# QingYunA/General-Medical-Image-Segmentation-CNN-Framework

Hardware: AMD Instinct MI355X
Metric: train voxels/sec (128^3 patches) 3D U-Net (higher is better)
Workload: dtype f32 (f16x3 split MFMA: every fp32 conv operand = two fp16 parts under a per-tensor power-of-two scale, three fp16 products per fp32 product, fp32 accumulate; graded against fp64 by the same tests as bf16x6 and the exact-fp32 MFMA path); 1 GPU; unet3d_f32_2x128: UNet3D(1,2,32) fwd+BCE+bwd+Adam+Dice, x=[2,1,128,128,128] fp32 per GPU, random-init (kaiming) weights, data-parallel replicas with RCCL gradient all-reduce, conv math f16x3; global_batch=2, parallelism=dp1, conv_math=f16x3, optimizer=torch.optim.Adam(fused=True)

## Files before the change

general-medical-image-segmentation-cnn-framework_amd/csrc/conv_mfma.hip:

```cpp
#include "common.h"
#include "internal.h"
#include "igemm_kernel.h"
#include "pack.h"
#include <stdlib.h>
#include <initializer_list>

namespace seg {

__global__ void pack_wq_kernel(const float* __restrict__ w, float* __restrict__ wq, int K, int Nn, int T, int NT, int mode, int aux, int CK,
                               int TW, TapList taps, const float* __restrict__ oscale) {
    const long long total = (long long)K * Nn * T;
    for (long long idx = (long long)blockIdx.x * blockDim.x + threadIdx.x; idx < total; idx += (long long)gridDim.x * blockDim.x) {
        long long r = idx;
        int s = (int)(r % 4); r /= 4;
        int j = (int)(r % NT); r /= NT;
        int h = (int)(r % 2); r /= 2;
        int kk = (int)(r % (CK / 8)); r /= (CK / 8);
        int tap = (int)(r % T); r /= T;
        int chunk = (int)(r % (K / CK)); r /= (K / CK);
        int nt = (int)r;
        wq[idx] = pack_src(w, mode, nt * NT + j, chunk * CK + kk * 8 + h * 4 + s, tap, K, Nn, T, aux, TW, taps) * (oscale ? oscale[nt * NT + j] : 1.f);
    }
}

__global__ void pack_wq_x3s_kernel(const float* __restrict__ w, bf16* __restrict__ wq, int K, int Nn, int NBW, int mode, const float* __restrict__ oscale) {
    const int NT = 32 * NBW, NU = X3S_NPAIR * NBW, nch = K / 16;
    const long long total = (long long)(Nn / NT) * nch * NU * 1024;
    for (long long idx = (long long)blockIdx.x * blockDim.x + threadIdx.x; idx < total; idx += (long long)gridDim.x * blockDim.x) {
        long long q = idx;
        const int e = (int)(q % 8); q /= 8;
        const int lane = (int)(q % 64); q /= 64;
        const int t2 = (int)(q % 2); q /= 2;
        const int u = (int)(q % NU); q /= NU;
        const int chunk = (int)(q % nch); q /= nch;
        const int nt = (int)q;
        const int s = u / NBW, nh = u % NBW, g = lane >> 4, c = lane & 15;
        const int tap = x3s_pair_tap(s, g >> 1);
        const int co = nt * NT + nh * 32 + t2 * 16 + c;
        const float v = tap < 27 ? pack_src(w, mode, co, chunk * 16 + 8 * (g & 1) + e, tap, K, Nn, 27, 0, 27, TapList{}) * (oscale ? oscale[co] : 1.f) : 0.f;
        bf16 bh, bm, bl;
        split3(v, bh, bm, bl);
        const long long base = (((long long)nt * nch + chunk) * NU + u) * 3072 + t2 * 512 + lane * 8 + e;
        wq[base] = bh; wq[base + 1024] = bm; wq[base + 2048] = bl;
    }
}

__global__ void pack_wq_x3s_f16_kernel(const float* __restrict__ w, _Float16* __restrict__ wq, int K, int Nn, int NBW, int mode, const float* __restrict__ oscale,
                                       const float* __restrict__ amax_w) {
    const int NT = 32 * NBW, NU = X3S_NPAIR * NBW, nch = K / 16;
    const long long total = (long long)(Nn / NT) * nch * NU * 1024;
    const float sc = pow2f(f16x_scale_exp(*amax_w));
    for (long long idx = (long long)blockIdx.x * blockDim.x + threadIdx.x; idx < total; idx += (long long)gridDim.x * blockDim.x) {
        long long q = idx;
        const int e = (int)(q % 8); q /= 8;
        const int lane = (int)(q % 64); q /= 64;
        const int t2 = (int)(q % 2); q /= 2;
        const int u = (int)(q % NU); q /= NU;
        const int chunk = (int)(q % nch); q /= nch;
        const int nt = (int)q;
        const int s = u / NBW, nh = u % NBW, g = lane >> 4, c = lane & 15;
        const int tap = x3s_pair_tap(s, g >> 1);
        const int co = nt * NT + nh * 32 + t2 * 16 + c;
        const float v = tap < 27 ? pack_src(w, mode, co, chunk * 16 + 8 * (g & 1) + e, tap, K, Nn, 27, 0, 27, TapList{}) * (oscale ? oscale[co] : 1.f) * sc : 0.f;
        _Float16 bh, bl;
        split2h(v, bh, bl);
        const long long base = (((long long)nt * nch + chunk) * NU + u) * 2048 + t2 * 512 + lane * 8 + e;
        wq[base] = bh; wq[base + 1024] = bl;
    }
}

__global__ __launch_bounds__(256) void amax_kernel(const float* __restrict__ x, int ld, long long rows, int C, const float* __restrict__ rowscale, unsigned* __restrict__ slot) {
    float m = 0.f;
    if ((C % 4) == 0 && (ld % 4) == 0 && ((uintptr_t)x % 16) == 0) {
        const int cw = C / 4;
        const long long total = rows * cw;
        for (long long idx = (long long)blockIdx.x * 256 + threadIdx.x; idx < total; idx += (long long)gridDim.x * 256) {
            const long long r = idx / cw;
            const f32x4_t v = *reinterpret_cast<const f32x4_t*>(x + r * ld + (idx - r * cw) * 4);
            const float sc = rowscale ? fabsf(rowscale[r]) : 1.f;
            m = fmaxf(m, fmaxf(fmaxf(fabsf(v[0]), fabsf(v[1])), fmaxf(fabsf(v[2]), fabsf(v[3]))) * sc);
        }
    } else {
        const long long total = rows * C;
        for (long long idx = (long long)blockIdx.x * 256 + threadIdx.x; idx < total; idx += (long long)gridDim.x * 256) {
            const long long r = idx / C;
            m = fmaxf(m, fabsf(x[r * ld + (idx - r * C)]) * (rowscale ? fabsf(rowscale[r]) : 1.f));
        }
    }
#pragma unroll
    for (int o = 32; o > 0; o >>= 1) m = fmaxf(m, __shfl_xor(m, o, 64));
    __shared__ float sh[4];
    if ((threadIdx.x & 63) == 0) sh[threadIdx.x >> 6] = m;
    __syncthreads();
    if (threadIdx.x == 0) {
        m = fmaxf(fmaxf(sh[0], sh[1]), fmaxf(sh[2], sh[3]));
        atomicMax(slot, __builtin_bit_cast(unsigned, m));
    }
}
void tensor_amax(const float* x, int ld, long long rows, int C, const float* rowscale, float* slot, hipStream_t st) {
    const long long work = rows * (long long)C / 4;
    const int grid = (int)(work / 1024 < 1 ? 1 : (work / 1024 > 2048 ? 2048 : work / 1024));
    hipLaunchKernelGGL(amax_kernel, dim3(grid), dim3(256), 0, st, x, ld, rows, C, rowscale, reinterpret_cast<unsigned*>(slot));
}

__global__ void pack_wq_b16s_kernel(const float* __restrict__ w, bf16* __restrict__ wq, int K, int Nn, int T, int NT, int mode, const float* __restrict__ oscale) {
    const int nstep = (T + 1) / 2, nch = K / 16, ntt = NT / 16;
    const long long total = (long long)(Nn / NT) * nch * nstep * ntt * 512;
    for (long long idx = (long long)blockIdx.x * blockDim.x + threadIdx.x; idx < total; idx += (long long)gridDim.x * blockDim.x) {
        long long q = idx;
        const int e = (int)(q % 8); q /= 8;
        const int lane = (int)(q % 64); q /= 64;
        const int tt = (int)(q % ntt); q /= ntt;
        const int s = (int)(q % nstep); q /= nstep;
        const int chunk = (int)(q % nch); q /= nch;
        const int nt = (int)q;
        const int g = lane >> 4, c = lane & 15;
        const int tap = 2 * s + (g >> 1);
        const int co = nt * NT + 32 * (tt >> 1) + 8 * (c >> 2) + 4 * (tt & 1) + (c & 3);
        wq[idx] = tap < T ? (bf16)(pack_src(w, mode, co, chunk * 16 + 8 * (g & 1) + e, tap, K, Nn, T, 0, T, TapList{}) * (oscale ? oscale[co] : 1.f)) : (bf16)0.f;
    }
// ... 592 lines not shown
```

general-medical-image-segmentation-cnn-framework_amd/csrc/conv_x3s.hip:

```cpp
#include "common.h"
#include "internal.h"
#include "igemm_kernel.h"
#include <type_traits>

namespace seg {

namespace {

#ifndef X3S_WN2
#define X3S_WN2 1
#endif
#ifndef X3S_WD
#define X3S_WD 3
#endif
#ifndef X3S_XD
#define X3S_XD 2
#endif
#ifndef X3S_HALO_AUX
#define X3S_HALO_AUX 0
#endif
#ifndef X3S_SPLIT_MIX
#define X3S_SPLIT_MIX 0
#endif
#ifndef X3S_BNX_EARLY
#define X3S_BNX_EARLY 1
#endif
constexpr int XBX = 16, XTY = 4, XHX = XBX + 2, XHY = XTY + 2;
constexpr int X3S_PRO_MAX_CIN = 512;

template <int LW, bool F16 = false, int WN = 1>
struct Geo {
    static constexpr int NPL = F16 ? 2 : 3;
    static constexpr int LINES = (4 / WN) * LW, TZ = LINES / XTY, HZ = TZ + 2;
    static constexpr int NVOX = XHX * XHY * HZ;
    static constexpr int PS = (NVOX + 15) / 16 * 16;
    static constexpr int LDS_BYTES = 2 * NPL * PS * 16;
    static constexpr int NPIECE = NVOX * 4;
    static constexpr int NITER = (NPIECE + 255) / 256;
};


__device__ __forceinline__ constexpr int tap_slot(int t) { return ((t / 9) * XHY + (t / 3) % 3) * XHX + t % 3; }
__device__ __forceinline__ constexpr int pair_kind(int s) { return s < 9 ? 0 : (s < 12 ? 1 : (s == 12 ? 2 : 3)); }

__device__ __forceinline__ float row16_sum(float v) {
    v += __builtin_bit_cast(float, __builtin_amdgcn_update_dpp(0, __builtin_bit_cast(int, v), 0xB1, 0xF, 0xF, true));
    v += __builtin_bit_cast(float, __builtin_amdgcn_update_dpp(0, __builtin_bit_cast(int, v), 0x4E, 0xF, 0xF, true));
    v += __builtin_bit_cast(float, __builtin_amdgcn_update_dpp(0, __builtin_bit_cast(int, v), 0x141, 0xF, 0xF, true));
    v += __builtin_bit_cast(float, __builtin_amdgcn_update_dpp(0, __builtin_bit_cast(int, v), 0x140, 0xF, 0xF, true));
    return v;
}

template <int LW, int NBW, int TZ, int WN = 1>
__device__ __forceinline__ void x3_epilogue(const IgemmArgs& a, f32x4 (&acc)[LW][2 * NBW], int scale_exp, int ks, int mtile, int n, int x0, int y0, int z0,
                                            int n0_tile, int line0, int r, int g, int wave, int tid, unsigned char* lds_raw) {
    constexpr int NT = 32 * NBW, NTW = 2 * NBW;
    constexpr int NTT = NT * WN, WM = 4 / WN;
    const int wn = WN == 1 ? 0 : wave % WN;
    const int n0 = n0_tile + wn * NT;
    const int gx = x0 + r;
    constexpr int LH = (8 / NTW) < LW ? (8 / NTW) : LW;
    constexpr int NG = (LW + LH - 1) / LH;
    constexpr bool DB = NG > 1 && NTW <= 2;
    f32x4 bxv[DB ? 2 : 1][LH][NTW];
    const int bnx_lane = min(gx, a.W - 1) * a.ldbnx + n0 + 4 * g;
    auto load_bnx = [&](int j0, int buf) {
#pragma unroll
        for (int j = 0; j < LH; ++j) {
            const int line = line0 + min(j0 + j, LW - 1);
            const int cz = min(z0 + line / XTY, a.D - 1), cy = min(y0 + line % XTY, a.H - 1);
            const float* src = a.bnx + (((long long)n * a.D + cz) * a.H + cy) * a.W * a.ldbnx + bnx_lane;
#pragma unroll
            for (int t = 0; t < NTW; ++t) bxv[buf][j][t] = *reinterpret_cast<const f32x4*>(src + 16 * t);
        }
    };
    if (a.bnpart) { load_bnx(0, 0); if (DB && X3S_BNX_EARLY) load_bnx(LH, 1); }
    if (scale_exp != 0) {
#pragma unroll
        for (int j = 0; j < LW; ++j)
#pragma unroll
            for (int t = 0; t < NTW; ++t)
#pragma unroll
                for (int e = 0; e < 4; ++e) acc[j][t][e] = __builtin_ldexpf(acc[j][t][e], scale_exp);
    }
    float* yslab = reinterpret_cast<float*>(a.y) + (long long)ks * a.split_stride;
    float* const ylane = yslab + ((((long long)n * a.D + z0) * a.H + y0) * a.W + gx) * a.ldy + n0 + 4 * g;
    float ssum[NTW][4];
#pragma unroll
    for (int t = 0; t < NTW; ++t)
#pragma unroll
        for (int e = 0; e < 4; ++e) ssum[t][e] = 0.f;
    float ymax = 0.f;
    f32x4 bv[NTW];
#pragma unroll
    for (int t = 0; t < NTW; ++t) bv[t] = a.bias ? *reinterpret_cast<const f32x4*>(a.bias + n0 + 16 * t + 4 * g) : f32x4{0.f, 0.f, 0.f, 0.f};
    auto store_lines = [&](auto ACTc) {
// ... 95 lines not shown
            for (int e = 0; e < 4; ++e) {
                const int c = 16 * t + 4 * g + e;
                float sm = 0.f;
#pragma unroll
                for (int w = 0; w < WM; ++w) sm += lds[(w * WN + wn) * NT + c];
                tmean[t][e] = sm / cnt;
            }
        __syncthreads();
        float m2[NTW][4];
#pragma unroll
        for (int t = 0; t < NTW; ++t)
#pragma unroll
            for (int e = 0; e < 4; ++e) m2[t][e] = 0.f;
#pragma unroll
        for (int j = 0; j < LW; ++j) {
            const int line = line0 + j;
            const bool inside = (z0 + line / XTY) < a.D && (y0 + line % XTY) < a.H && gx < a.W;
#pragma unroll
            for (int t = 0; t < NTW; ++t)
#pragma unroll
                for (int e = 0; e < 4; ++e) {
                    const float d = acc[j][t][e] + bv[t][e] - tmean[t][e];
                    if (inside) m2[t][e] += d * d;
                }
        }
#pragma unroll
        for (int t = 0; t < NTW; ++t)
#pragma unroll
            for (int e = 0; e < 4; ++e) {
                const float v = row16_sum(m2[t][e]);
                if (r == 0) lds[(4 + wave) * NT + 16 * t + 4 * g + e] = v;
            }
        __syncthreads();
        if (tid < NTT) {
            const int cw = tid / NT, cl = tid % NT;
            float s1 = 0.f, mm = 0.f;
#pragma unroll
            for (int w = 0; w < WM; ++w) { s1 += lds[(w * WN + cw) * NT + cl]; mm += lds[(4 + w * WN + cw) * NT + cl]; }
            float* dst = a.spart + ((long long)mtile * a.Cout + n0_tile + tid) * 3;
            dst[0] = s1; dst[1] = mm; dst[2] = cnt;
        }
    }
}

template <int LW, int NBW, bool F16, int WN = 1, bool PRO = false>
__global__ __launch_bounds__(256, 2) void conv_x3s_kernel(IgemmArgs a) {
    using G = Geo<LW, F16, WN>;
    constexpr int NPL = G::NPL;
    constexpr int NT = 32 * NBW * WN;
    constexpr int NTW = 2 * NBW;
    constexpr int NU = X3S_NPAIR * NBW;
    constexpr int NUP = X3S_NPAIR * NBW * WN;
    constexpr int UNIT = 2 * NPL * 512;
    constexpr int PS = G::PS;
    extern __shared__ __attribute__((aligned(16))) unsigned char lds_raw[];

    const int tid = threadIdx.x, lane = tid & 63, wave = __builtin_amdgcn_readfirstlane(tid >> 6);
    const int r = lane & 15, g = lane >> 4;

    int ks, ntile, mtile, n, x0, y0, z0;
    {
        const int total = (int)gridDim.x, bid = blockIdx.x;
        const int q8 = total >> 3, r8 = total & 7, xcd = bid & 7;
        const int xstart = xcd < r8 ? xcd * (q8 + 1) : r8 * (q8 + 1) + (xcd - r8) * q8, xcnt = q8 + (xcd < r8 ? 1 : 0);
        const int local = bid >> 3;
        if (local >= xcnt) return;
        int t = xstart + local;
        ks = t % a.ksplit; t /= a.ksplit;
        ntile = t % a.nN;
        mtile = t / a.nN;
        int mt = mtile;
        const int per_n = a.ntx * a.nty * a.ntz;
        n = mt / per_n; mt -= n * per_n;
        const int zfull = a.ntz / a.bz;
        const int rowtiles = a.ntx * a.nty * a.bz;
        int zrow = mt / rowtiles, bzz = a.bz;
        if (zrow >= zfull) { zrow = zfull; bzz = a.ntz - zfull * a.bz; }
        mt -= zrow * rowtiles;
        const int blk = a.ntx * a.by * bzz;
        const int b = mt / blk; mt -= b * blk;
        const int txi = mt % a.ntx; mt /= a.ntx;
        const int tyi = b * a.by + mt % a.by;
        const int tzi = zrow * a.bz + mt / a.by;
        x0 = txi * XBX; y0 = tyi * XTY; z0 = tzi * G::TZ;
    }
    const int n0 = ntile * NT;
    const int c0 = ks * a.cps, c1 = c0 + a.cps;
    const float* __restrict__ xin = reinterpret_cast<const float*>(a.x);
    int sx = 0, sw = 0;
    if constexpr (F16) { sx = f16x_scale_exp(*a.amax_x); sw = f16x_scale_exp(*a.amax_w); }
    const float xscale = pow2f(sx);
    float* const ptab = reinterpret_cast<float*>(lds_raw + G::LDS_BYTES);
    const int pcin = a.nchunks * 16;
    if constexpr (PRO) {
        for (int i = tid; i < pcin; i += 256) { ptab[i] = a.pro_al[i] * xscale; ptab[pcin + i] = a.pro_be[i] * xscale; }
    }

    int voff[G::NITER];
    halo_piece_offsets<G::NITER, G::NPIECE, 4, XHX, XHY, G::HZ>(voff, tid, x0 - 1, y0 - 1, z0 - 1, a.D, a.H, a.W, a.ldx * 4);
    const float* xsample = xin + (long long)n * a.D * a.H * a.W * a.ldx;
    const int sample_bytes = a.D * a.H * a.W * a.ldx * 4;
    f32x4 stage[G::NITER];
    auto load_stage = [&](int chunk) {
        const auto rsrc = __builtin_amdgcn_make_buffer_rsrc(const_cast<float*>(xsample + chunk * 16), 0, sample_bytes, 0x00020000);
#pragma unroll
        for (int it = 0; it < G::NITER; ++it)
// ... 29 lines not shown
#endif
    unsigned char* const wdst = lds_raw + (((tid & 3) >> 1) * PS + (tid >> 2)) * 16 + (tid & 1) * 8;
    auto write_stage = [&](int chunk, auto WPRO, auto MASK, auto RELU) {
        f32x4 pal = {0.f, 0.f, 0.f, 0.f}, pbe = pal;
        if constexpr (decltype(WPRO)::value) {
            pal = *reinterpret_cast<const f32x4*>(ptab + chunk * 16 + (tid & 3) * 4);
            pbe = *reinterpret_cast<const f32x4*>(ptab + pcin + chunk * 16 + (tid & 3) * 4);
        }
#pragma unroll
        for (int it = 0; it < G::NITER; ++it) {
            if (it * 256 + tid < G::NPIECE) {
                using u32x2 = __attribute__((ext_vector_type(2))) unsigned;
                unsigned char* dst = wdst + it * 1024;
                if constexpr (F16) {
                    unsigned h0, l0, h1, l1;
                    if constexpr (decltype(WPRO)::value) {
                        f32x4 v;
#pragma unroll
                        for (int e = 0; e < 4; ++e) {
                            const float z = fmaf(stage[it][e], pal[e], pbe[e]);
                            v[e] = decltype(RELU)::value ? fmaxf(z, 0.f) : fmaxf(z, z * a.pro_slope);
                        }
                        if constexpr (decltype(MASK)::value) { if (voff[it] == 0x7FFFFFF0) v = f32x4{0.f, 0.f, 0.f, 0.f}; }
                        split_pair_h(v[0], v[1], h0, l0, 1.f);
                        split_pair_h(v[2], v[3], h1, l1, 1.f);
                    } else if (SEG_DBG(a, 256)) {
                        using u32x4 = __attribute__((ext_vector_type(4))) unsigned;
                        const u32x4 u = __builtin_bit_cast(u32x4, stage[it]);
                        h0 = u[0]; h1 = u[1]; l0 = u[2]; l1 = u[3];
                    } else {
                        split_pair_h(stage[it][0], stage[it][1], h0, l0, xscale);
                        split_pair_h(stage[it][2], stage[it][3], h1, l1, xscale);
                    }
                    const u32x2 qh = {h0, h1}, ql = {l0, l1};
                    *reinterpret_cast<u32x2*>(dst) = qh;
                    *reinterpret_cast<u32x2*>(dst + 2 * PS * 16) = ql;
                } else {
                    unsigned h0, m0, l0, h1, m1, l1;
                    split_pair(stage[it][0], stage[it][1], h0, m0, l0);
                    split_pair(stage[it][2], stage[it][3], h1, m1, l1);
                    const u32x2 qh = {h0, h1}, qm = {m0, m1}, ql = {l0, l1};
                    *reinterpret_cast<u32x2*>(dst) = qh;
                    *reinterpret_cast<u32x2*>(dst + 2 * PS * 16) = qm;
                    *reinterpret_cast<u32x2*>(dst + 4 * PS * 16) = ql;
                }
            }
        }
    };

    const int wm = WN == 1 ? wave : wave / WN, wn = WN == 1 ? 0 : wave % WN;
    const int line0 = wm * LW;
    const int lane_slot = ((line0 / XTY) * XHY + (line0 % XTY)) * XHX + r + (g & 1) * PS;
    const int hi = g >> 1;
    const int xb0 = (lane_slot + hi) * 16, xb1 = (lane_slot + hi * XHX) * 16, xb2 = (lane_slot + hi * XHY * XHX) * 16, xb3 = lane_slot * 16;
    auto xaddr = [&](int s, int j, int pl) {
        const int base = pair_kind(s) == 0 ? xb0 : (pair_kind(s) == 1 ? xb1 : (pair_kind(s) == 2 ? xb2 : xb3));
        return base + (((j >> 2) * XHY + (j & 3)) * XHX + tap_slot(x3s_pair_tap(s, 0)) + 2 * pl * PS) * 16;
    };

    f32x4 acc[LW][NTW];
#pragma unroll
    for (int j = 0; j < LW; ++j)
#pragma unroll
        for (int t = 0; t < NTW; ++t) acc[j][t] = f32x4{0.f, 0.f, 0.f, 0.f};
    const bool interior = x0 >= 1 && y0 >= 1 && z0 >= 1 && x0 + XBX + 1 <= a.W && y0 + XTY + 1 <= a.H && z0 + G::TZ + 1 <= a.D;

    const bf16* wlane = reinterpret_cast<const bf16*>(a.wq) + (long long)ntile * a.nchunks * (NUP * UNIT) + lane * 8;
    if (!SEG_DBG(a, 1024)) load_stage(c0);
    for (int chunk = c0; chunk < (SEG_DBG(a, 512) ? c0 : c1); ++chunk) {
        const bf16* wp = wlane + (long long)chunk * (NUP * UNIT) + wn * (NBW * UNIT);
        constexpr int WD = F16 ? ((PRO && LW == 8 && WN == 1) ? 2 : X3S_WD) : (NBW == 2 && LW == 4 ? 1 : 2);
        constexpr int XD = F16 ? X3S_XD : 1;
        bf16x8_t wf[WD + 1][2][NPL], xf[XD + 1][NPL];
        auto load_w = [&](int u) {
#pragma unroll
            for (int t2 = 0; t2 < 2; ++t2)
#pragma unroll
                for (int pl = 0; pl < NPL; ++pl) wf[u % (WD + 1)][t2][pl] = *reinterpret_cast<const bf16x8_t*>(wp + ((u / NBW) * (NBW * WN) + u % NBW) * UNIT + (pl * 2 + t2) * 512);
        };
#pragma unroll
        for (int u = 0; u < WD; ++u) load_w(u);
        if (!SEG_DBG(a, 1) || chunk == c0) {
        __syncthreads();
        if (!SEG_DBG(a, 4) || chunk == c0) {
            using TT = std::true_type; using FF = std::false_type;
            if constexpr (!PRO) write_stage(chunk, FF{}, FF{}, FF{});
            else if (a.pro_act == MI355SEG_ACT_RELU) { if (interior) write_stage(chunk, TT{}, FF{}, TT{}); else write_stage(chunk, TT{}, TT{}, TT{}); }
            else write_stage(chunk, TT{}, TT{}, FF{});
        }
        __syncthreads();
        }
        const bool more = chunk + 1 < c1;
#pragma unroll
        for (int q0 = 0; q0 < XD; ++q0)
#pragma unroll
            for (int pl = 0; pl < NPL; ++pl) xf[q0][pl] = *reinterpret_cast<const bf16x8_t*>(lds_raw + xaddr((q0 / LW) / NBW, q0 % LW, pl));
        __builtin_amdgcn_sched_barrier(0);
#pragma unroll
        for (int u = 0; u < NU; ++u) {
            const int s = u / NBW, nh = u % NBW;
#pragma unroll
            for (int j = 0; j < LW; ++j) {
                const int q = u * LW + j, cur = q % (XD + 1), nxt = (q + XD) % (XD + 1);
                if (j == 0 && u + WD < NU && !SEG_DBG(a, 2)) load_w(u + WD);
                if (q < G::NITER && more && !SEG_DBG(a, 1) && !SEG_DBG(a, 16)) load_piece(chunk + 1, q);
                if (q + XD < NU * LW && !SEG_DBG(a, 8)) {
                    const int u2 = (q + XD) / LW, j2 = (q + XD) % LW;
#pragma unroll
                    for (int pl = 0; pl < NPL; ++pl) xf[nxt][pl] = *reinterpret_cast<const bf16x8_t*>(lds_raw + xaddr(u2 / NBW, j2, pl));
                }
                if constexpr (F16) {
                    constexpr int PW[3] = {1, 0, 0}, PX[3] = {0, 1, 0};
#pragma unroll
                    for (int pr = 0; pr < 3; ++pr)
#pragma unroll
                        for (int t2 = 0; t2 < 2; ++t2)
                            acc[j][nh * 2 + t2] = __builtin_amdgcn_mfma_f32_16x16x32_f16(__builtin_bit_cast(f16x8_t, wf[u % (WD + 1)][t2][PW[pr]]),
                                                                                      __builtin_bit_cast(f16x8_t, xf[cur][PX[pr]]), acc[j][nh * 2 + t2], 0, 0, 0);
                } else {
                    constexpr int PW[6] = {2, 0, 1, 1, 0, 0}, PX[6] = {0, 2, 1, 0, 1, 0};
#pragma unroll
                    for (int pr = 0; pr < 6; ++pr)
#pragma unroll
                        for (int t2 = 0; t2 < 2; ++t2)
                            acc[j][nh * 2 + t2] = __builtin_amdgcn_mfma_f32_16x16x32_bf16(wf[u % (WD + 1)][t2][PW[pr]], xf[cur][PX[pr]], acc[j][nh * 2 + t2], 0, 0, 0);
                }
#pragma unroll
                for (int k = 0; k < NPL; ++k) {
                    __builtin_amdgcn_sched_group_barrier(0x100, 1, 0);
                    __builtin_amdgcn_sched_group_barrier(0x008, 1, 0);
                }
                if (j == 0 || q < G::NITER) {
#pragma unroll
                    for (int k = 0; k < 2 * NPL + 1; ++k) {
                        __builtin_amdgcn_sched_group_barrier(0x020, 1, 0);
                        __builtin_amdgcn_sched_group_barrier(0x008, 1, 0);
                    }
                }
                __builtin_amdgcn_sched_barrier(0);
            }
        }
        __builtin_amdgcn_sched_barrier(0);
    }

    x3_epilogue<LW, NBW, G::TZ, WN>(a, acc, F16 ? -(sx + sw) : 0, ks, mtile, n, x0, y0, z0, n0, line0, r, g, wave, tid, lds_raw);
}

template <int LW, int NBW, bool F16, int WN = 1>
void launch_x3s(const IgemmArgs& a, int nwg, hipStream_t st) {
    constexpr int LDSB = Geo<LW, F16, WN>::LDS_BYTES;
    static_assert(LDSB >= 8 * 64 * 4, "the statistics epilogue needs 8 x NT floats");
    if constexpr (F16) {
        if (a.pro_al) {
            SEG_SET_LDS((conv_x3s_kernel<LW, NBW, true, WN, true>), LDSB + X3S_PRO_MAX_CIN * 8);
            hipLaunchKernelGGL((conv_x3s_kernel<LW, NBW, true, WN, true>), dim3(nwg), dim3(256), LDSB + a.nchunks * 16 * 8, st, a);
            return;
        }
    }
    SEG_SET_LDS((conv_x3s_kernel<LW, NBW, F16, WN>), LDSB);
    hipLaunchKernelGGL((conv_x3s_kernel<LW, NBW, F16, WN>), dim3(nwg), dim3(256), LDSB, st, a);
}


template <int NBW>
struct GeoW {
    static constexpr int LW = 8, TZ = 8, HZ = TZ + 2;
    static constexpr int NVOX = XHX * XHY * HZ;
    static constexpr int PS = (NVOX + 15) / 16 * 16;
    static constexpr int BUF = 4 * PS * 16;
    static constexpr int LDS_BYTES = 2 * BUF;
    static constexpr int NPIECE = NVOX * 4;
    static constexpr int NITER = (NPIECE + 255) / 256;
    static constexpr int NCH = NBW == 2 ? 1 : 2;
    static constexpr int WR = NBW == 2 ? 2 : 4, WL = NBW == 2 ? 1 : 2;
    static constexpr int RING = 8;
    static_assert((NCH * X3S_NPAIR) % WR == 0 && WL < WR, "the weight ring's phase must be static");
};

// ... 30 lines not shown
        const int txi = mt % a.ntx; mt /= a.ntx;
        const int tyi = b * a.by + mt % a.by;
        const int tzi = zrow * a.bz + mt / a.by;
        x0 = txi * XBX; y0 = tyi * XTY; z0 = tzi * G::TZ;
    }
    const int n0 = ntile * NT;
    const int c1 = a.cps;
    const float* __restrict__ xin = reinterpret_cast<const float*>(a.x);
    const int sx = f16x_scale_exp(*a.amax_x), sw = f16x_scale_exp(*a.amax_w);
    const float xscale = pow2f(sx);

    int voff[NITER];
#pragma unroll
    for (int it = 0; it < NITER; ++it) {
        const int p = it * 256 + tid;
        const int vox = p >> 2, part = p & 3;
        const int hz = vox / (XHY * XHX), rem = vox % (XHY * XHX);
        const int hy = rem / XHX, hx = rem % XHX;
        const int gz = z0 - 1 + hz, gy = y0 - 1 + hy, gx = x0 - 1 + hx;
        const bool ok = (p < G::NPIECE) && (unsigned)gz < (unsigned)a.D && (unsigned)gy < (unsigned)a.H && (unsigned)gx < (unsigned)a.W;
        voff[it] = ok ? (((gz * a.H + gy) * a.W + gx) * a.ldx + part * 4) * 4 : 0x7FFFFFF0;
    }
    const float* xsample = xin + (long long)n * a.D * a.H * a.W * a.ldx;
    const int sample_bytes = a.D * a.H * a.W * a.ldx * 4;
    f32x4 ring[RING];
    auto load_piece = [&](int chunk, int it) {
        const auto rsrc = __builtin_amdgcn_make_buffer_rsrc(const_cast<float*>(xsample + chunk * 16), 0, sample_bytes, 0x00020000);
        ring[it % RING] = __builtin_bit_cast(f32x4, __builtin_amdgcn_raw_buffer_load_b128(rsrc, voff[it], 0, X3S_HALO_AUX));
    };
    auto split_pair_h = [&](float x0_, float x1_, unsigned& h2, unsigned& l2) {
        const float s0 = x0_ * xscale, s1 = x1_ * xscale;
        const f16x2_t hh = __builtin_convertvector(f32x2_t{s0, s1}, f16x2_t);
        h2 = __builtin_bit_cast(unsigned, hh);
        const float r0 = __builtin_fmaf((float)hh[0], -1.f, s0), r1 = __builtin_fmaf((float)hh[1], -1.f, s1);
        l2 = __builtin_bit_cast(unsigned, __builtin_convertvector(f32x2_t{r0, r1}, f16x2_t));
    };
    unsigned char* const wdst = lds_raw + (((tid & 3) >> 1) * PS + (tid >> 2)) * 16 + (tid & 1) * 8;
    auto write_piece = [&](int buf, int it) {
        if (it * 256 + tid < G::NPIECE) {
            using u32x2 = __attribute__((ext_vector_type(2))) unsigned;
            const f32x4 v = ring[it % RING];
            unsigned h0, l0, h1, l1;
            split_pair_h(v[0], v[1], h0, l0);
            split_pair_h(v[2], v[3], h1, l1);
            unsigned char* dst = wdst + buf * G::BUF + it * 1024;
            *reinterpret_cast<u32x2*>(dst) = u32x2{h0, h1};
            *reinterpret_cast<u32x2*>(dst + 2 * PS * 16) = u32x2{l0, l1};
        }
    };

    const int line0 = wave * LW;
    const int lane_slot = ((line0 / XTY) * XHY + (line0 % XTY)) * XHX + r + (g & 1) * PS;
    const int hi = g >> 1;
    const int xb0 = (lane_slot + hi) * 16, xb1 = (lane_slot + hi * XHX) * 16, xb2 = (lane_slot + hi * XHY * XHX) * 16, xb3 = lane_slot * 16;
    auto xoffs = [](int buf, int s, int j, int pl) {
        return buf * G::BUF + ((((j >> 2) * XHY + (j & 3)) * XHX + tap_slot(x3s_pair_tap(s, 0))) + 2 * pl * PS) * 16;
    };

    f32x4 acc[LW][NTW];
#pragma unroll
    for (int j = 0; j < LW; ++j)
#pragma unroll
        for (int t = 0; t < NTW; ++t) acc[j][t] = f32x4{0.f, 0.f, 0.f, 0.f};

    const _Float16* wlane = reinterpret_cast<const _Float16*>(a.wq) + (long long)ntile * a.nchunks * (NS * STEP) + lane * 8;
    const int nlin = c1 * NS;
    bf16x8_t wf[G::WR][NTW][2];
    auto load_w_frag = [&](int slot, int lin, int f) {
        const int t = f >> 1, pl = f & 1;
        wf[slot][t][pl] = *reinterpret_cast<const bf16x8_t*>(wlane + (long long)lin * STEP + (t >> 1) * 2048 + pl * 1024 + (t & 1) * 512);
    };

#pragma unroll
    for (int sl = 0; sl < G::WL; ++sl)
#pragma unroll
        for (int f = 0; f < 2 * NTW; ++f) load_w_frag(sl, sl < nlin ? sl : 0, f);
#pragma unroll
    for (int it0 = 0; it0 < NITER; it0 += RING) {
#pragma unroll
        for (int it = it0; it < it0 + RING && it < NITER; ++it) load_piece(0, it);
#pragma unroll
        for (int it = it0; it < it0 + RING && it < NITER; ++it) write_piece(0, it);
    }
    __syncthreads();

    bf16x8_t xf[2][2];
    for (int chunk = 0; chunk < c1; chunk += G::NCH) {
#pragma unroll
        for (int h = 0; h < G::NCH; ++h) {
            const int cur = G::NCH == 2 ? h : (chunk & 1);
            const int cbuf = G::NCH == 2 ? h : 0;
            const int rt = G::NCH == 2 ? 0 : cur * G::BUF;
            const int nbuf = 1 - cur;
            const bool more = chunk + h + 1 < c1;
            const int b0 = xb0 + rt, b1 = xb1 + rt, b2 = xb2 + rt, b3 = xb3 + rt;
            const unsigned char* xl = lds_raw;
#pragma unroll
            for (int pl = 0; pl < 2; ++pl) xf[0][pl] = *reinterpret_cast<const bf16x8_t*>(xl + b0 + xoffs(cbuf, 0, 0, pl));
            __builtin_amdgcn_sched_barrier(0);
#pragma unroll
            for (int s = 0; s < NS; ++s) {
                const int hs = h * NS + s;
                const int lin = (chunk + h) * NS + s;
#pragma unroll
                for (int j = 0; j < LW; ++j) {
                    const int q = s * LW + j, cb = q & 1, nb = cb ^ 1;
                    {
                        constexpr int FPL = (2 * NTW + LW - 1) / LW;
#pragma unroll
                        for (int f = j * FPL; f < (j + 1) * FPL && f < 2 * NTW; ++f) {
                            const int l2 = lin + G::WL;
                            load_w_frag((hs + G::WL) % G::WR, l2 < nlin ? l2 : nlin - 1, f);
                        }
                    }
                    if (q >= RING && q - RING < NITER && more) write_piece(nbuf, q - RING);
                    if (q < NITER && more) load_piece(chunk + h + 1, q);
                    if (q + 1 < NS * LW) {
                        const int s2 = (q + 1) / LW, j2 = (q + 1) % LW;
#pragma unroll
                        for (int pl = 0; pl < 2; ++pl)
                            xf[nb][pl] = *reinterpret_cast<const bf16x8_t*>(xl + (pair_kind(s2) == 0 ? b0 : (pair_kind(s2) == 1 ? b1 : (pair_kind(s2) == 2 ? b2 : b3))) + xoffs(cbuf, s2, j2, pl));
                    }
                    constexpr int PW[3] = {1, 0, 0}, PX[3] = {0, 1, 0};
#pragma unroll
                    for (int pr = 0; pr < 3; ++pr)
#pragma unroll
                        for (int t = 0; t < NTW; ++t)
                            acc[j][t] = __builtin_amdgcn_mfma_f32_16x16x32_f16(__builtin_bit_cast(f16x8_t, wf[hs % G::WR][t][PW[pr]]),
                                                                            __builtin_bit_cast(f16x8_t, xf[cb][PX[pr]]), acc[j][t], 0, 0, 0);
#pragma unroll
                    for (int k = 0; k < 2; ++k) {
                        __builtin_amdgcn_sched_group_barrier(0x100, 1, 0);
                        __builtin_amdgcn_sched_group_barrier(0x008, 1, 0);
                    }
#pragma unroll
                    for (int k = 0; k < 2; ++k) {
                        __builtin_amdgcn_sched_group_barrier(0x020, 1, 0);
                        __builtin_amdgcn_sched_group_barrier(0x008, 1, 0);
                    }
                    __builtin_amdgcn_sched_barrier(0);
                }
            }
            __syncthreads();
        }
    }

    x3_epilogue<LW, NBW, G::TZ>(a, acc, -(sx + sw), 0, mtile, n, x0, y0, z0, n0, line0, r, g, wave, tid, lds_raw);
}

template <int NBW>
void launch_x3w(const IgemmArgs& a, int nwg, hipStream_t st) {
    constexpr int LDSB = GeoW<NBW>::LDS_BYTES;
    SEG_SET_LDS((conv_x3w_kernel<NBW>), LDSB);
    hipLaunchKernelGGL((conv_x3w_kernel<NBW>), dim3(nwg), dim3(256), LDSB, st, a);
}

}

bool x3s_plan_ok(const IgemmPlan& p, const void* x, int ldx, const void* y, int ldy, long long sample_voxels) {
    if (sample_voxels * ldx * 4 >= 0x7FFFFFF0LL) return false;
    return p.KS == 3 && p.CK == 16 && p.BX == 16 && (p.MB == 1 || p.MB == 2) && (p.NBW == 1 || p.NBW == 2) && p.WN == 1 && p.TY == 4 &&
           (ldx % 4) == 0 && (ldy % 4) == 0 && ((uintptr_t)x % 16) == 0 && ((uintptr_t)y % 16) == 0;
}

bool x3w_plan(IgemmPlan& p, int N, int D, int H, int W, int Cin, int Cout, int ksplit) {
#ifdef MI355SEG_TUNE
    static const char* off = getenv("MI355SEG_NO_X3W");
    if (off && off[0] == '1') return false;
#endif
    if (ksplit != 1 || p.WN != 1 || p.NBW != 1) return false;
    const int ntz = (D + 7) / 8, nty = (H + 3) / 4, ntx = (W + 15) / 16;
    const long long tiles = (long long)N * ntz * nty * ntx * p.nN;
    if (tiles < 512 || (double)(ntz * 8) / D > 1.15) return false;
    p.MB = 4; p.TZ = 8; p.ntx = ntx; p.nty = nty; p.ntz = ntz; p.nM = N * ntz * nty * ntx;
    return true;
}

void dispatch_x3s(const IgemmPlan& p, const IgemmArgs& a, int nwg, hipStream_t st) {
    if (a.amax_x && p.MB == 4) {
#ifdef X3W_NBW1
        if (p.NBW == 2) launch_x3w<2>(a, nwg, st); else launch_x3w<1>(a, nwg, st);
#else
// ... 15 lines not shown
```

general-medical-image-segmentation-cnn-framework_amd/csrc/prepack.hip:

```cpp
#include "common.h"
#include "internal.h"
#include "igemm_kernel.h"
#include "pack.h"
#include <algorithm>
#include <cstring>
#include <mutex>
#include <vector>

namespace seg {

namespace {

template <int LAYOUT, int NB>
__device__ __forceinline__ void pack_tiled_body(const int vbid, float* tile, const float* __restrict__ w, bf16* __restrict__ wq, int K, int Nn, int T, int P, int mode,
                                                const float* __restrict__ oscale, const float* __restrict__ amax_w) {
    const int nnb = Nn / NB;
    const int n0 = (vbid % nnb) * NB, chunk = vbid / nnb, k0 = chunk * 16;
    const int tid = threadIdx.x;
    const int nrun = mode == 0 ? NB : 16, rlen = (mode == 0 ? 16 : NB) * T;
    for (int i = tid * 4; i < nrun * rlen; i += 1024) {
        const int run = i / rlen, off = i - run * rlen;
        const float* src = mode == 0 ? w + ((long long)(n0 + run) * K + k0) * T : w + ((long long)(k0 + run) * Nn + n0) * T;
        *reinterpret_cast<f32x4_t*>(tile + i) = *reinterpret_cast<const f32x4_t*>(src + off);
    }
    __syncthreads();
    const int nstep = LAYOUT == 0 ? (T + 1) / 2 : X3S_NPAIR, nch = K / 16;
    constexpr int LB = NB == 8 ? 3 : (NB == 4 ? 2 : 1);
    for (int q = tid; q < nstep * 4 * NB; q += 256) {
        const int half = q & 1, nl = (q >> 1) & (NB - 1), gh = (q >> (1 + LB)) & 1, s = q >> (2 + LB);
        const int tap = LAYOUT == 0 ? 2 * s + gh : x3s_pair_tap(s, gh);
        const int n = n0 + nl, g = 2 * gh + half;
        float v[8];
        if (tap < T) {
            float sc = (oscale && mode == 0) ? oscale[n] : 1.f;
            if (LAYOUT == 2) sc *= pow2f(f16x_scale_exp(*amax_w));
#pragma unroll
            for (int e = 0; e < 8; ++e) {
                const int kl = 8 * half + e;
                v[e] = (mode == 0 ? tile[(nl * 16 + kl) * T + tap] : tile[(kl * NB + nl) * T + (T - 1 - tap)]) * sc;
            }
        } else {
#pragma unroll
            for (int e = 0; e < 8; ++e) v[e] = 0.f;
        }
        if (LAYOUT == 0) {
            const int NT = P, ntt = NT / 16, nt = n / NT, nin = n - nt * NT;
            const int tt = 2 * (nin / 32) + ((nin >> 2) & 1), c = 4 * ((nin & 31) >> 3) + (nin & 3);
            bf16x8_t o;
#pragma unroll
            for (int e = 0; e < 8; ++e) o[e] = (bf16)v[e];
            reinterpret_cast<bf16x8_t*>(wq)[((((long long)nt * nch + chunk) * nstep + s) * ntt + tt) * 64 + c + 16 * g] = o;
        } else if (LAYOUT == 2) {
            const int NBW = P, NT = 32 * NBW, nt = n / NT, nin = n - nt * NT;
            const int nh = nin / 32, t2 = (nin & 31) >> 4, c = nin & 15;
            f16x8_t oh, ol;
#pragma unroll
            for (int e = 0; e < 8; ++e) { _Float16 a, b; split2h(v[e], a, b); oh[e] = a; ol[e] = b; }
            _Float16* dst = reinterpret_cast<_Float16*>(wq) + (((long long)nt * nch + chunk) * (X3S_NPAIR * NBW) + s * NBW + nh) * 2048 + t2 * 512 + (c + 16 * g) * 8;
            *reinterpret_cast<f16x8_t*>(dst) = oh;
            *reinterpret_cast<f16x8_t*>(dst + 1024) = ol;
        } else {
            const int NBW = P, NT = 32 * NBW, nt = n / NT, nin = n - nt * NT;
            const int nh = nin / 32, t2 = (nin & 31) >> 4, c = nin & 15;
            bf16x8_t oh, om, ol;
#pragma unroll
            for (int e = 0; e < 8; ++e) { bf16 a, b, d; split3(v[e], a, b, d); oh[e] = a; om[e] = b; ol[e] = d; }
            bf16* dst = wq + (((long long)nt * nch + chunk) * (X3S_NPAIR * NBW) + s * NBW + nh) * 3072 + t2 * 512 + (c + 16 * g) * 8;
            *reinterpret_cast<bf16x8_t*>(dst) = oh;
            *reinterpret_cast<bf16x8_t*>(dst + 1024) = om;
            *reinterpret_cast<bf16x8_t*>(dst + 2048) = ol;
        }
    }
}

template <int NP, typename IDX>
__device__ __forceinline__ void pack_wq_lowp_body(const int vbid, const int nvb, const float* __restrict__ w, bf16* __restrict__ wq, int K, int Nn, int T, int NT, int mode,
                                                  int aux, int CK, int TW, const TapList& taps, const float* __restrict__ oscale) {
    const IDX total = (IDX)K * Nn * T;
    const int plane = 2 * NT * 8;
    for (IDX idx = (IDX)vbid * blockDim.x + threadIdx.x; idx < total; idx += (IDX)nvb * blockDim.x) {
        IDX r = idx;
        const int e = (int)(r % 8); r /= 8;
        const int j = (int)(r % NT); r /= NT;
        const int h = (int)(r % 2); r /= 2;
        const int kst = (int)(r % (CK / 16)); r /= (CK / 16);
        const int tap = (int)(r % T); r /= T;
        const int chunk = (int)(r % (K / CK)); r /= (K / CK);
        const int nt = (int)r;
        const float v = pack_src(w, mode, nt * NT + j, chunk * CK + kst * 16 + 8 * h + e, tap, K, Nn, T, aux, TW, taps) * (oscale ? oscale[nt * NT + j] : 1.f);
        const long long base = ((((long long)nt * (K / CK) + chunk) * T + tap) * (CK / 16) + kst) * (NP * plane) + ((long long)h * NT + j) * 8 + e;
        if (NP == 3) {
            bf16 bh, bm, bl;
            split3(v, bh, bm, bl);
            wq[base] = bh; wq[base + plane] = bm; wq[base + 2 * plane] = bl;
        } else {
            wq[base] = (bf16)v;
        }
    }
}

template <int NP>
__device__ __forceinline__ void convt_pack_planes_body(const int vbid, const int nvb, const float* __restrict__ w, bf16x8_t* __restrict__ wq, int Cin, int Cout,
                                                       int gather, int BN, int K, int Ncols) {
    const int nchunk = K / 64;
    const long long total = (long long)(Ncols / BN) * nchunk * 8 * BN;
    for (long long i = (long long)vbid * blockDim.x + threadIdx.x; i < total; i += (long long)nvb * blockDim.x) {
        const int row = (int)(i % BN); long long q = i / BN;
        const int kgp = (int)(q % 8); q /= 8;
        const int chunk = (int)(q % nchunk); const int ntile = (int)(q / nchunk);
        const int n = ntile * BN + row, k0 = chunk * 64 + kgp * 8;
        bf16x8_t ph, pm, pl;
#pragma unroll
        for (int e = 0; e < 8; ++e) {
            const int k = NP == 3 ? (k0 & ~31) + 4 * ((k0 >> 3) & 3) + (e < 4 ? e : 12 + e) : k0 + e;
            int ci, co, t;
            if (gather) { ci = n; t = k / Cout; co = k - t * Cout; }
            else { ci = k; t = n / Cout; co = n - t * Cout; }
            const float v = w[((long long)ci * Cout + co) * 8 + t];
            bf16 h, m, l;
            split3(v, h, m, l);
            ph[e] = h; pm[e] = m; pl[e] = l;
        }
        bf16x8_t* dst = wq + (((long long)ntile * nchunk + chunk) * NP * 8 + kgp) * BN + row;
// ... 268 lines not shown
```

Baseline: 219.1 million voxels/s.

## Use K=16 MFMA for the odd 27th tap instead of zero-padded K=32 pair

The 3x3x3 conv packs taps in pairs, so the 27th tap was previously paired with a zero tap and run through full 16x16x32 MFMAs. The last pair step now uses a repacked weight layout and half-width LDS loads, feeding 16x16x16 MFMAs over only the real tap. This removes wasted MFMA work on the zero half and halves the weight and activation fragment traffic for that step. In exchange it adds a new packed layout that every packer and both kernel variants must agree on, plus extra branching in the unrolled inner loop.

```diff
diff --git a/general-medical-image-segmentation-cnn-framework_amd/csrc/conv_mfma.hip b/general-medical-image-segmentation-cnn-framework_amd/csrc/conv_mfma.hip
--- a/general-medical-image-segmentation-cnn-framework_amd/csrc/conv_mfma.hip
+++ b/general-medical-image-segmentation-cnn-framework_amd/csrc/conv_mfma.hip
@@ -35,13 +35,21 @@
         const int chunk = (int)(q % nch); q /= nch;
         const int nt = (int)q;
         const int s = u / NBW, nh = u % NBW, g = lane >> 4, c = lane & 15;
-        const int tap = x3s_pair_tap(s, g >> 1);
+        const bool odd = s == X3S_NPAIR - 1;
+        const int tap = odd ? 26 : x3s_pair_tap(s, g >> 1);
         const int co = nt * NT + nh * 32 + t2 * 16 + c;
-        const float v = tap < 27 ? pack_src(w, mode, co, chunk * 16 + 8 * (g & 1) + e, tap, K, Nn, 27, 0, 27, TapList{}) * (oscale ? oscale[co] : 1.f) : 0.f;
+        const int ci = chunk * 16 + (odd ? 4 * g + e : 8 * (g & 1) + e);
+        const float v = (!odd || e < 4) ? pack_src(w, mode, co, ci, tap, K, Nn, 27, 0, 27, TapList{}) * (oscale ? oscale[co] : 1.f) : 0.f;
         bf16 bh, bm, bl;
         split3(v, bh, bm, bl);
-        const long long base = (((long long)nt * nch + chunk) * NU + u) * 3072 + t2 * 512 + lane * 8 + e;
-        wq[base] = bh; wq[base + 1024] = bm; wq[base + 2048] = bl;
+        const long long unit = (((long long)nt * nch + chunk) * NU + u) * 3072;
+        if (odd) {
+            const long long base = unit + (e < 4 ? 0 : 1536) + lane * 8 + t2 * 4 + (e & 3);
+            wq[base] = bh; wq[base + 512] = bm; wq[base + 1024] = bl;
+        } else {
+            const long long base = unit + t2 * 512 + lane * 8 + e;
+            wq[base] = bh; wq[base + 1024] = bm; wq[base + 2048] = bl;
+        }
     }
 }
 
@@ -59,13 +67,21 @@
         const int chunk = (int)(q % nch); q /= nch;
         const int nt = (int)q;
         const int s = u / NBW, nh = u % NBW, g = lane >> 4, c = lane & 15;
-        const int tap = x3s_pair_tap(s, g >> 1);
+        const bool odd = s == X3S_NPAIR - 1;
+        const int tap = odd ? 26 : x3s_pair_tap(s, g >> 1);
         const int co = nt * NT + nh * 32 + t2 * 16 + c;
-        const float v = tap < 27 ? pack_src(w, mode, co, chunk * 16 + 8 * (g & 1) + e, tap, K, Nn, 27, 0, 27, TapList{}) * (oscale ? oscale[co] : 1.f) * sc : 0.f;
+        const int ci = chunk * 16 + (odd ? 4 * g + e : 8 * (g & 1) + e);
+        const float v = (!odd || e < 4) ? pack_src(w, mode, co, ci, tap, K, Nn, 27, 0, 27, TapList{}) * (oscale ? oscale[co] : 1.f) * sc : 0.f;
         _Float16 bh, bl;
         split2h(v, bh, bl);
-        const long long base = (((long long)nt * nch + chunk) * NU + u) * 2048 + t2 * 512 + lane * 8 + e;
-        wq[base] = bh; wq[base + 1024] = bl;
+        const long long unit = (((long long)nt * nch + chunk) * NU + u) * 2048;
+        if (odd) {
+            const long long base = unit + (e < 4 ? 0 : 1024) + lane * 8 + t2 * 4 + (e & 3);
+            wq[base] = bh; wq[base + 512] = bl;
+        } else {
+            const long long base = unit + t2 * 512 + lane * 8 + e;
+            wq[base] = bh; wq[base + 1024] = bl;
+        }
     }
 }
 
diff --git a/general-medical-image-segmentation-cnn-framework_amd/csrc/conv_x3s.hip b/general-medical-image-segmentation-cnn-framework_amd/csrc/conv_x3s.hip
--- a/general-medical-image-segmentation-cnn-framework_amd/csrc/conv_x3s.hip
+++ b/general-medical-image-segmentation-cnn-framework_amd/csrc/conv_x3s.hip
@@ -42,6 +42,11 @@
 
 __device__ __forceinline__ constexpr int tap_slot(int t) { return ((t / 9) * XHY + (t / 3) % 3) * XHX + t % 3; }
 __device__ __forceinline__ constexpr int pair_kind(int s) { return s < 9 ? 0 : (s < 12 ? 1 : (s == 12 ? 2 : 3)); }
+
+typedef short s16x4_t __attribute__((ext_vector_type(4)));
+__device__ __forceinline__ bf16x8_t widen4(bf16x4_t v) { return __builtin_shufflevector(v, v, 0, 1, 2, 3, -1, -1, -1, -1); }
+__device__ __forceinline__ bf16x4_t low4(bf16x8_t v) { return __builtin_shufflevector(v, v, 0, 1, 2, 3); }
+__device__ __forceinline__ bf16x4_t half4(bf16x8_t v, int hi) { return hi ? __builtin_shufflevector(v, v, 4, 5, 6, 7) : low4(v); }
 
 __device__ __forceinline__ float row16_sum(float v) {
     v += __builtin_bit_cast(float, __builtin_amdgcn_update_dpp(0, __builtin_bit_cast(int, v), 0xB1, 0xF, 0xF, true));
@@ -243,6 +248,7 @@
     constexpr int NU = X3S_NPAIR * NBW;
     constexpr int NUP = X3S_NPAIR * NBW * WN;
     constexpr int UNIT = 2 * NPL * 512;
+    constexpr int SODD = X3S_NPAIR - 1;
     constexpr int PS = G::PS;
     extern __shared__ __attribute__((aligned(16))) unsigned char lds_raw[];
 
@@ -378,7 +384,8 @@
     const int line0 = wm * LW;
     const int lane_slot = ((line0 / XTY) * XHY + (line0 % XTY)) * XHX + r + (g & 1) * PS;
     const int hi = g >> 1;
-    const int xb0 = (lane_slot + hi) * 16, xb1 = (lane_slot + hi * XHX) * 16, xb2 = (lane_slot + hi * XHY * XHX) * 16, xb3 = lane_slot * 16;
+    const int xb0 = (lane_slot + hi) * 16, xb1 = (lane_slot + hi * XHX) * 16, xb2 = (lane_slot + hi * XHY * XHX) * 16;
+    const int xb3 = (lane_slot - (g & 1) * PS + hi * PS) * 16 + (g & 1) * 8;
     auto xaddr = [&](int s, int j, int pl) {
         const int base = pair_kind(s) == 0 ? xb0 : (pair_kind(s) == 1 ? xb1 : (pair_kind(s) == 2 ? xb2 : xb3));
         return base + (((j >> 2) * XHY + (j & 3)) * XHX + tap_slot(x3s_pair_tap(s, 0)) + 2 * pl * PS) * 16;
@@ -402,7 +409,18 @@
 #pragma unroll
             for (int t2 = 0; t2 < 2; ++t2)
 #pragma unroll
-                for (int pl = 0; pl < NPL; ++pl) wf[u % (WD + 1)][t2][pl] = *reinterpret_cast<const bf16x8_t*>(wp + ((u / NBW) * (NBW * WN) + u % NBW) * UNIT + (pl * 2 + t2) * 512);
+                for (int pl = 0; pl < NPL; ++pl) {
+                    const bf16* src = wp + ((u / NBW) * (NBW * WN) + u % NBW) * UNIT;
+                    if (u / NBW == SODD) { if (t2 == 0) wf[u % (WD + 1)][0][pl] = *reinterpret_cast<const bf16x8_t*>(src + pl * 512); }
+                    else wf[u % (WD + 1)][t2][pl] = *reinterpret_cast<const bf16x8_t*>(src + (pl * 2 + t2) * 512);
+                }
+        };
+        auto load_x = [&](int slot, int s, int j) {
+#pragma unroll
+            for (int pl = 0; pl < NPL; ++pl) {
+                if (s == SODD) xf[slot][pl] = widen4(*reinterpret_cast<const bf16x4_t*>(lds_raw + xaddr(s, j, pl)));
+                else xf[slot][pl] = *reinterpret_cast<const bf16x8_t*>(lds_raw + xaddr(s, j, pl));
+            }
         };
 #pragma unroll
         for (int u = 0; u < WD; ++u) load_w(u);
@@ -418,9 +436,7 @@
         }
         const bool more = chunk + 1 < c1;
 #pragma unroll
-        for (int q0 = 0; q0 < XD; ++q0)
-#pragma unroll
-            for (int pl = 0; pl < NPL; ++pl) xf[q0][pl] = *reinterpret_cast<const bf16x8_t*>(lds_raw + xaddr((q0 / LW) / NBW, q0 % LW, pl));
+        for (int q0 = 0; q0 < XD; ++q0) load_x(q0, (q0 / LW) / NBW, q0 % LW);
         __builtin_amdgcn_sched_barrier(0);
 #pragma unroll
         for (int u = 0; u < NU; ++u) {
@@ -432,24 +448,33 @@
                 if (q < G::NITER && more && !SEG_DBG(a, 1) && !SEG_DBG(a, 16)) load_piece(chunk + 1, q);
                 if (q + XD < NU * LW && !SEG_DBG(a, 8)) {
                     const int u2 = (q + XD) / LW, j2 = (q + XD) % LW;
-#pragma unroll
-                    for (int pl = 0; pl < NPL; ++pl) xf[nxt][pl] = *reinterpret_cast<const bf16x8_t*>(lds_raw + xaddr(u2 / NBW, j2, pl));
+                    load_x(nxt, u2 / NBW, j2);
                 }
                 if constexpr (F16) {
                     constexpr int PW[3] = {1, 0, 0}, PX[3] = {0, 1, 0};
 #pragma unroll
                     for (int pr = 0; pr < 3; ++pr)
 #pragma unroll
-                        for (int t2 = 0; t2 < 2; ++t2)
-                            acc[j][nh * 2 + t2] = __builtin_amdgcn_mfma_f32_16x16x32_f16(__builtin_bit_cast(f16x8_t, wf[u % (WD + 1)][t2][PW[pr]]),
-                                                                                      __builtin_bit_cast(f16x8_t, xf[cur][PX[pr]]), acc[j][nh * 2 + t2], 0, 0, 0);
+                        for (int t2 = 0; t2 < 2; ++t2) {
+                            if (s == SODD)
+                                acc[j][nh * 2 + t2] = __builtin_amdgcn_mfma_f32_16x16x16f16(__builtin_bit_cast(f16x4_t, half4(wf[u % (WD + 1)][0][PW[pr]], t2)),
+                                                                                         __builtin_bit_cast(f16x4_t, low4(xf[cur][PX[pr]])), acc[j][nh * 2 + t2], 0, 0, 0);
+                            else
+                                acc[j][nh * 2 + t2] = __builtin_amdgcn_mfma_f32_16x16x32_f16(__builtin_bit_cast(f16x8_t, wf[u % (WD + 1)][t2][PW[pr]]),
+                                                                                          __builtin_bit_cast(f16x8_t, xf[cur][PX[pr]]), acc[j][nh * 2 + t2], 0, 0, 0);
+                        }
                 } else {
                     constexpr int PW[6] = {2, 0, 1, 1, 0, 0}, PX[6] = {0, 2, 1, 0, 1, 0};
 #pragma unroll
                     for (int pr = 0; pr < 6; ++pr)
 #pragma unroll
-                        for (int t2 = 0; t2 < 2; ++t2)
-                            acc[j][nh * 2 + t2] = __builtin_amdgcn_mfma_f32_16x16x32_bf16(wf[u % (WD + 1)][t2][PW[pr]], xf[cur][PX[pr]], acc[j][nh * 2 + t2], 0, 0, 0);
+                        for (int t2 = 0; t2 < 2; ++t2) {
+                            if (s == SODD)
+                                acc[j][nh * 2 + t2] = __builtin_amdgcn_mfma_f32_16x16x16bf16_1k(__builtin_bit_cast(s16x4_t, half4(wf[u % (WD + 1)][0][PW[pr]], t2)),
+                                                                                             __builtin_bit_cast(s16x4_t, low4(xf[cur][PX[pr]])), acc[j][nh * 2 + t2], 0, 0, 0);
+                            else
+                                acc[j][nh * 2 + t2] = __builtin_amdgcn_mfma_f32_16x16x32_bf16(wf[u % (WD + 1)][t2][PW[pr]], xf[cur][PX[pr]], acc[j][nh * 2 + t2], 0, 0, 0);
+                        }
                 }
 #pragma unroll
                 for (int k = 0; k < NPL; ++k) {
@@ -586,8 +611,9 @@
     const int line0 = wave * LW;
     const int lane_slot = ((line0 / XTY) * XHY + (line0 % XTY)) * XHX + r + (g & 1) * PS;
     const int hi = g >> 1;
-    const int xb0 = (lane_slot + hi) * 16, xb1 = (lane_slot + hi * XHX) * 16, xb2 = (lane_slot + hi * XHY * XHX) * 16, xb3 = lane_slot * 16;
-    auto xoffs = [](int buf, int s, int j, int pl) {
+    const int xb0 = (lane_slot + hi) * 16, xb1 = (lane_slot + hi * XHX) * 16, xb2 = (lane_slot + hi * XHY * XHX) * 16;
+    const int xb3 = (lane_slot - (g & 1) * PS + hi * PS) * 16 + (g & 1) * 8;
+    auto xoffs =[](int buf, int s, int j, int pl) {
         return buf * G::BUF + ((((j >> 2) * XHY + (j & 3)) * XHX + tap_slot(x3s_pair_tap(s, 0))) + 2 * pl * PS) * 16;
     };
 
@@ -600,15 +626,16 @@
     const _Float16* wlane = reinterpret_cast<const _Float16*>(a.wq) + (long long)ntile * a.nchunks * (NS * STEP) + lane * 8;
     const int nlin = c1 * NS;
     bf16x8_t wf[G::WR][NTW][2];
-    auto load_w_frag = [&](int slot, int lin, int f) {
+    auto load_w_frag = [&](int slot, int lin, int f, bool odd) {
         const int t = f >> 1, pl = f & 1;
-        wf[slot][t][pl] = *reinterpret_cast<const bf16x8_t*>(wlane + (long long)lin * STEP + (t >> 1) * 2048 + pl * 1024 + (t & 1) * 512);
+        if (!odd) wf[slot][t][pl] = *reinterpret_cast<const bf16x8_t*>(wlane + (long long)lin * STEP + (t >> 1) * 2048 + pl * 1024 + (t & 1) * 512);
+        else if ((t & 1) == 0) wf[slot][t][pl] = *reinterpret_cast<const bf16x8_t*>(wlane + (long long)lin * STEP + (t >> 1) * 2048 + pl * 512);
     };
 
 #pragma unroll
     for (int sl = 0; sl < G::WL; ++sl)
 #pragma unroll
-        for (int f = 0; f < 2 * NTW; ++f) load_w_frag(sl, sl < nlin ? sl : 0, f);
+        for (int f = 0; f < 2 * NTW; ++f) load_w_frag(sl, sl < nlin ? sl : 0, f, false);
 #pragma unroll
     for (int it0 = 0; it0 < NITER; it0 += RING) {
 #pragma unroll
@@ -644,7 +671,7 @@
 #pragma unroll
                         for (int f = j * FPL; f < (j + 1) * FPL && f < 2 * NTW; ++f) {
                             const int l2 = lin + G::WL;
-                            load_w_frag((hs + G::WL) % G::WR, l2 < nlin ? l2 : nlin - 1, f);
+                            load_w_frag((hs + G::WL) % G::WR, l2 < nlin ? l2 : nlin - 1, f, (s + G::WL) % NS == NS - 1);
                         }
                     }
                     if (q >= RING && q - RING < NITER && more) write_piece(nbuf, q - RING);
@@ -652,16 +679,24 @@
                     if (q + 1 < NS * LW) {
                         const int s2 = (q + 1) / LW, j2 = (q + 1) % LW;
 #pragma unroll
-                        for (int pl = 0; pl < 2; ++pl)
-                            xf[nb][pl] = *reinterpret_cast<const bf16x8_t*>(xl + (pair_kind(s2) == 0 ? b0 : (pair_kind(s2) == 1 ? b1 : (pair_kind(s2) == 2 ? b2 : b3))) + xoffs(cbuf, s2, j2, pl));
+                        for (int pl = 0; pl < 2; ++pl) {
+                            const unsigned char* src = xl + (pair_kind(s2) == 0 ? b0 : (pair_kind(s2) == 1 ? b1 : (pair_kind(s2) == 2 ? b2 : b3))) + xoffs(cbuf, s2, j2, pl);
+                            if (s2 == NS - 1) xf[nb][pl] = widen4(*reinterpret_cast<const bf16x4_t*>(src));
+                            else xf[nb][pl] = *reinterpret_cast<const bf16x8_t*>(src);
+                        }
                     }
                     constexpr int PW[3] = {1, 0, 0}, PX[3] = {0, 1, 0};
 #pragma unroll
                     for (int pr = 0; pr < 3; ++pr)
 #pragma unroll
-                        for (int t = 0; t < NTW; ++t)
-                            acc[j][t] = __builtin_amdgcn_mfma_f32_16x16x32_f16(__builtin_bit_cast(f16x8_t, wf[hs % G::WR][t][PW[pr]]),
-                                                                            __builtin_bit_cast(f16x8_t, xf[cb][PX[pr]]), acc[j][t], 0, 0, 0);
+                        for (int t = 0; t < NTW; ++t) {
+                            if (s == NS - 1)
+                                acc[j][t] = __builtin_amdgcn_mfma_f32_16x16x16f16(__builtin_bit_cast(f16x4_t, half4(wf[hs % G::WR][t & ~1][PW[pr]], t & 1)),
+                                                                               __builtin_bit_cast(f16x4_t, low4(xf[cb][PX[pr]])), acc[j][t], 0, 0, 0);
+                            else
+                                acc[j][t] = __builtin_amdgcn_mfma_f32_16x16x32_f16(__builtin_bit_cast(f16x8_t, wf[hs % G::WR][t][PW[pr]]),
+                                                                                __builtin_bit_cast(f16x8_t, xf[cb][PX[pr]]), acc[j][t], 0, 0, 0);
+                        }
 #pragma unroll
                     for (int k = 0; k < 2; ++k) {
                         __builtin_amdgcn_sched_group_barrier(0x100, 1, 0);
diff --git a/general-medical-image-segmentation-cnn-framework_amd/csrc/prepack.hip b/general-medical-image-segmentation-cnn-framework_amd/csrc/prepack.hip
--- a/general-medical-image-segmentation-cnn-framework_amd/csrc/prepack.hip
+++ b/general-medical-image-segmentation-cnn-framework_amd/csrc/prepack.hip
@@ -28,10 +28,19 @@
     constexpr int LB = NB == 8 ? 3 : (NB == 4 ? 2 : 1);
     for (int q = tid; q < nstep * 4 * NB; q += 256) {
         const int half = q & 1, nl = (q >> 1) & (NB - 1), gh = (q >> (1 + LB)) & 1, s = q >> (2 + LB);
-        const int tap = LAYOUT == 0 ? 2 * s + gh : x3s_pair_tap(s, gh);
+        const bool odd = LAYOUT != 0 && s == X3S_NPAIR - 1;
+        const int tap = LAYOUT == 0 ? 2 * s + gh : (odd ? 26 : x3s_pair_tap(s, gh));
         const int n = n0 + nl, g = 2 * gh + half;
         float v[8];
-        if (tap < T) {
+        if (odd) {
+            float sc = (oscale && mode == 0) ? oscale[n] : 1.f;
+            if (LAYOUT == 2) sc *= pow2f(f16x_scale_exp(*amax_w));
+#pragma unroll
+            for (int e = 0; e < 8; ++e) {
+                const int kl = 4 * g + (e & 3);
+                v[e] = e < 4 ? (mode == 0 ? tile[(nl * 16 + kl) * T + tap] : tile[(kl * NB + nl) * T + (T - 1 - tap)]) * sc : 0.f;
+            }
+        } else if (tap < T) {
             float sc = (oscale && mode == 0) ? oscale[n] : 1.f;
             if (LAYOUT == 2) sc *= pow2f(f16x_scale_exp(*amax_w));
 #pragma unroll
@@ -56,19 +65,40 @@
             f16x8_t oh, ol;
 #pragma unroll
             for (int e = 0; e < 8; ++e) { _Float16 a, b; split2h(v[e], a, b); oh[e] = a; ol[e] = b; }
-            _Float16* dst = reinterpret_cast<_Float16*>(wq) + (((long long)nt * nch + chunk) * (X3S_NPAIR * NBW) + s * NBW + nh) * 2048 + t2 * 512 + (c + 16 * g) * 8;
-            *reinterpret_cast<f16x8_t*>(dst) = oh;
-            *reinterpret_cast<f16x8_t*>(dst + 1024) = ol;
+            _Float16* unit = reinterpret_cast<_Float16*>(wq) + (((long long)nt * nch + chunk) * (X3S_NPAIR * NBW) + s * NBW + nh) * 2048;
+            if (odd) {
+                _Float16* dst = unit + (c + 16 * g) * 8 + t2 * 4;
+#pragma unroll
+                for (int hf = 0; hf < 2; ++hf) {
+                    *reinterpret_cast<f16x4_t*>(dst + hf * 1024) = f16x4_t{oh[4 * hf], oh[4 * hf + 1], oh[4 * hf + 2], oh[4 * hf + 3]};
+                    *reinterpret_cast<f16x4_t*>(dst + hf * 1024 + 512) = f16x4_t{ol[4 * hf], ol[4 * hf + 1], ol[4 * hf + 2], ol[4 * hf + 3]};
+                }
+            } else {
+                _Float16* dst = unit + t2 * 512 + (c + 16 * g) * 8;
+                *reinterpret_cast<f16x8_t*>(dst) = oh;
+                *reinterpret_cast<f16x8_t*>(dst + 1024) = ol;
+            }
         } else {
             const int NBW = P, NT = 32 * NBW, nt = n / NT, nin = n - nt * NT;
             const int nh = nin / 32, t2 = (nin & 31) >> 4, c = nin & 15;
             bf16x8_t oh, om, ol;
 #pragma unroll
             for (int e = 0; e < 8; ++e) { bf16 a, b, d; split3(v[e], a, b, d); oh[e] = a; om[e] = b; ol[e] = d; }
-            bf16* dst = wq + (((long long)nt * nch + chunk) * (X3S_NPAIR * NBW) + s * NBW + nh) * 3072 + t2 * 512 + (c + 16 * g) * 8;
-            *reinterpret_cast<bf16x8_t*>(dst) = oh;
-            *reinterpret_cast<bf16x8_t*>(dst + 1024) = om;
-            *reinterpret_cast<bf16x8_t*>(dst + 2048) = ol;
+            bf16* unit = wq + (((long long)nt * nch + chunk) * (X3S_NPAIR * NBW) + s * NBW + nh) * 3072;
+            if (odd) {
+                bf16* dst = unit + (c + 16 * g) * 8 + t2 * 4;
+#pragma unroll
+                for (int hf = 0; hf < 2; ++hf) {
+                    *reinterpret_cast<bf16x4_t*>(dst + hf * 1536) = bf16x4_t{oh[4 * hf], oh[4 * hf + 1], oh[4 * hf + 2], oh[4 * hf + 3]};
+                    *reinterpret_cast<bf16x4_t*>(dst + hf * 1536 + 512) = bf16x4_t{om[4 * hf], om[4 * hf + 1], om[4 * hf + 2], om[4 * hf + 3]};
+                    *reinterpret_cast<bf16x4_t*>(dst + hf * 1536 + 1024) = bf16x4_t{ol[4 * hf], ol[4 * hf + 1], ol[4 * hf + 2], ol[4 * hf + 3]};
+                }
+            } else {
+                bf16* dst = unit + t2 * 512 + (c + 16 * g) * 8;
+                *reinterpret_cast<bf16x8_t*>(dst) = oh;
+                *reinterpret_cast<bf16x8_t*>(dst + 1024) = om;
+                *reinterpret_cast<bf16x8_t*>(dst + 2048) = ol;
+            }
         }
     }
 }
```

Measured after the change: 220.0 million voxels/s, median of 6. About the same (+0.4%).
